# AssemblyAI-Community/MinImagen

Measured on NVIDIA H100. Metric: denoising steps/sec (SR256 U-Net, batch 32 per GPU per step), higher is better.
Workload: dtype f16 tensor-core operands, f32 accumulate / residual stream

## Files before the change

include/minimagen_b200.h:

```cpp
#ifndef MINIMAGEN_B200_H_
#define MINIMAGEN_B200_H_

#include <stdint.h>

#ifdef __cplusplus
extern "C" {
#endif

#define MI_ABI_VERSION 2

int mi_abi_version(void);
const char* mi_last_error(void);
int mi_device_ok(void);
int mi_set_launch_mode(int programmatic_dependent_launch);

int mi_pack_conv_weight_f16(const float* w_oihw, int c_out, int c_in, int kh, int kw, float scale, void* out_f16,
                            void* stream);

int mi_pack_conv_weight_dgrad_f16(const float* w_oihw, int c_out, int c_in, int kh, int kw, void* out_f16, void* stream);

int mi_conv2d_igemm_supported(int H, int W, int c_in, int c_out);
int mi_conv2d_igemm_f16(const void* act_f16, int B, int H, int W, int lda, int c_off, int c_in, const void* act2_f16,
                        int lda2, int c_off2, int c_in1, const void* w_f16, int c_out, int kh, int kw, int mode,
                        const float* bias, const float* residual, float* out_f32, void* out_f16, double* out_stats,
                        long long out_sb, long long out_sh, long long out_sw, long long out_sc, int n_valid,
                        int block_n, int* err_flag, void* workspace, long long workspace_bytes, void* stream);
int mi_conv3x3_res1x1_supported(int H, int W, int c_in, int c_out, int x_cin);
int mi_conv3x3_res1x1_f16(const void* act_f16, int B, int H, int W, int lda, int c_in, const void* act2_f16, int lda2,
                          int c_in1, const void* x_f16, int ldx, int x_cin, const void* x2_f16, int ldx2, int x_cin1,
                          const void* w_f16, int c_out, const float* bias, const float* residual, float* out_f32,
                          void* out_f16, double* out_stats, int* err_flag, void* stream);
long long mi_conv2d_igemm_workspace_bytes(void);

int mi_conv3x3_gn_supported(int H, int W, int c0, int c1, int c_out, int groups);
int mi_conv3x3_gn_silu_f16(const float* src0, int c0, const float* src1, int c1, float scale1, int B, int H, int W,
                           int groups, const double* stats0, const double* stats1, const float* gamma,
                           const float* beta, const float* scale_shift, int scale_shift_ld, float eps,
                           const void* w_f16, int c_out, const float* bias, const float* residual, float* out_f32,
                           void* out_f16, double* out_stats, int* err_flag, void* stream);

int mi_conv2d_direct_f32(const float* in, int B, int Hin, int Win, int c_in, int ldi, const float* w_oihw, int c_out,
                         int kh, int kw, int stride, int pad, const float* bias, const float* residual, float* out,
                         int Hout, int Wout, long long out_sb, long long out_sh, long long out_sw, long long out_sc,
                         void* stream);

int mi_gn_stats(const void* src0, int c0, const void* src1, int c1, float scale1, int in_is_f16, int B, int hw,
                int groups, double* sums, void* stream);
int mi_gn_apply_silu(const void* src0, int c0, const void* src1, int c1, float scale1, int in_is_f16, int B, int hw,
                     int groups, const double* stats0, int stats0_block, const double* stats1, int stats1_block,
                     const float* gamma, const float* beta, const float* scale_shift, int scale_shift_ld, float eps,
                     void* out, int out_is_f16, void* stream);
int mi_cast_act(const void* src0, int c0, const void* src1, int c1, float scale1, int in_is_f16, int B, int H, int W,
                int mode, void* out, int out_is_f16, void* stream);
int mi_ln_rows(const float* in, long long rows, int C, const float* gamma, const float* beta, float eps, int pre_gelu,
               const float* residual, float* out_f32, void* out_f16, void* stream);

int mi_linear_f32(const float* in, int M, int K, const float* W, const float* bias, int N, int in_act, int out_act,
                  const float* addend, float* out_f32, void* out_f16, float out_scale, void* stream);
int mi_sinusoidal_posemb(const long long* t, int B, int dim, float* out, void* stream);
int mi_text_tokens(const float* proj, int B, int L, int D, const uint8_t* mask, const uint8_t* keep,
                   const float* null_embed, int max_len, float* c_out, int m, int row_off, float* pooled,
                   void* stream);
// ... 83 lines not shown
```

minimagen_b200/csrc/capi.cu:

```cuda
#include "../../include/minimagen_b200.h"

#include <cuda_runtime.h>
#include <stdio.h>
#include <stdlib.h>
#include <string.h>
#include <string>

#include "conv_tc.cuh"
#include "kernels.cuh"

namespace {

thread_local char g_err[256] = "ok";

int fail(int code, const char* what) {
    snprintf(g_err, sizeof(g_err), "%s (code %d)", what, code);
    return code;
}
int check(int rc, const char* fn) {
    if (rc == 0) return 0;
    if (rc == -1) return fail(rc, (std::string(fn) + ": unsupported shape / alignment").c_str());
    if (rc == -2) {
        cudaError_t e = cudaGetLastError();
        return fail(rc, (std::string(fn) + ": kernel launch failed: " + cudaGetErrorString(e)).c_str());
    }
    return fail(rc, (std::string(fn) + ": error").c_str());
}
inline cudaStream_t S(void* s) { return reinterpret_cast<cudaStream_t>(s); }

}

namespace mi {
static bool g_pdl = false;
bool pdl_enabled() { return g_pdl; }
}

extern "C" {

int mi_abi_version(void) { return MI_ABI_VERSION; }
int mi_set_launch_mode(int programmatic_dependent_launch) {
    mi::g_pdl = programmatic_dependent_launch != 0;
    return 0;
}
const char* mi_last_error(void) { return g_err; }

int mi_device_ok(void) {
    int dev = 0, major = 0;
    if (cudaGetDevice(&dev) != cudaSuccess) return 0;
    if (cudaDeviceGetAttribute(&major, cudaDevAttrComputeCapabilityMajor, dev) != cudaSuccess) return 0;
    return major == 9;
}

int mi_pack_conv_weight_dgrad_f16(const float* w, int c_out, int c_in, int kh, int kw, void* out, void* stream) {
    return check(mi::pack_conv_weight_dgrad(w, c_out, c_in, kh, kw, (__half*)out, S(stream)), "mi_pack_conv_weight_dgrad_f16");
}
int mi_pack_conv_weight_f16(const float* w, int c_out, int c_in, int kh, int kw, float scale, void* out, void* stream) {
    return check(mi::pack_conv_weight(w, c_out, c_in, kh, kw, scale, (__half*)out, S(stream)), "mi_pack_conv_weight_f16");
}

int mi_conv2d_igemm_supported(int H, int W, int c_in, int c_out) { return mi::conv_tc_supported(H, W, c_in, c_out) ? 1 : 0; }

static int igemm_common(const void* act, int B, int H, int W, int lda, int c_off, int c_in, const void* act2, int lda2,
                        int c_off2, int c_in1, const void* w, int c_out, int kh, int kw, int mode, const float* bias,
                        const float* residual, float* out_f32, void* out_f16, double* out_stats, long long out_sb,
                        long long out_sh, long long out_sw, long long out_sc, int n_valid, int block_n, int* err_flag,
                        void* workspace, long long workspace_bytes, const void* x_act, int ldx, int x_off, int x_cin,
                        const void* x_act2, int ldx2, int x_off2, int x_cin1, void* stream) {
    mi::ConvTcProblem p{};
    p.x_act = x_act; p.x_lda = ldx; p.x_chan_off = x_off; p.Cx = x_cin;
    p.x_act2 = x_act2; p.x_lda2 = ldx2; p.x_chan_off2 = x_off2; p.Cx1 = x_cin1;
    if (x_act && !(mode == 0 && kh == 3 && kw == 3)) return fail(-9, "mi_conv3x3_res1x1_f16: the folded 1x1 operand needs a 3x3 stride-1 conv");
    (void)workspace; (void)workspace_bytes;
    p.act = act; p.B = B; p.H = H; p.W = W; p.lda = lda; p.a_channels = lda; p.a_chan_off = c_off; p.Cin = c_in;
    p.wpacked = w; p.Cout = c_out;
    p.act2 = act2; p.lda2 = lda2; p.a_chan_off2 = c_off2; p.Cin1 = c_in1; p.stats = out_stats;
    if (out_stats && (out_sc > 1 || (c_out % 32) != 0)) return fail(-8, "mi_conv2d_igemm_f16: out_stats needs channel-contiguous output and c_out % 32 == 0");
    if (out_stats && ((long long)H * W) % 32 != 0)
        return fail(-8, "mi_conv2d_igemm_f16: out_stats needs H*W % 32 == 0 (a warp's output rows must belong to one image)");
    p.out_f32 = out_f32; p.out_f16 = (__half*)out_f16; p.bias = bias; p.residual = residual;
    p.out_sb = out_sb; p.out_sh = out_sh; p.out_sw = out_sw; p.out_sc = out_sc; p.n_valid = n_valid;
    p.block_n_hint = block_n; p.err_flag = err_flag;
    if (mode == 0) {
        if (!(kh & 1) || !(kw & 1) || kh * kw > mi::kConvMaxTaps) return fail(-4, "mi_conv2d_igemm_f16: mode 0 needs odd kh,kw with kh*kw <= 16");
// ... 297 lines not shown
```

minimagen_b200/csrc/conv_tc.cu:

```cuda
#include "conv_tc.cuh"

#include <cuda_runtime.h>
#include <mutex>
#include <stdio.h>

#include "kernels.cuh"
#include "launch.cuh"
#include "ptx.cuh"
#include "sat_half.cuh"
#include "wgmma.cuh"

namespace mi {

namespace {

constexpr int kNumThreads = 384;
constexpr uint32_t kABytes = kConvBlockM * kConvBlockK * 2;
constexpr uint32_t kRingBudget = 192 * 1024;
constexpr uint32_t kAuxBytes = 512;
constexpr uint32_t kSmemMax = 227 * 1024;
constexpr int kProducerRegs = 40;
constexpr int kConsumerRegs = 232;
static_assert(128 * kProducerRegs + 256 * kConsumerRegs <= 65536, "register file overcommitted");
constexpr int kTurnBar = 2;
constexpr int kStatBar = 4;
constexpr uint32_t stat_scratch_bytes(int block_n) { return 2 * 4 * (block_n / 16 > 0 ? block_n / 16 : 1) * 2 * 8; }

template <int BLOCK_N>
struct Cfg {
    static constexpr uint32_t kBBytes = BLOCK_N * kConvBlockK * 2;
    static constexpr uint32_t kStageBytes = kABytes + kBBytes;
    static constexpr int kStages = (kRingBudget / kStageBytes) > 8 ? 8 : (kRingBudget / kStageBytes);
    static constexpr uint32_t kSmemBytes = kStages * kStageBytes + 1024  + kAuxBytes;
};

__device__ __forceinline__ float silu(float v) { return __fdividef(v, 1.0f + __expf(-v)); }

template <int BLOCK_N, bool GN>
__global__ void __launch_bounds__(kNumThreads, 1)
conv_wg_kernel(const __grid_constant__ CUtensorMap tmA, const __grid_constant__ CUtensorMap tmA2,
               const __grid_constant__ CUtensorMap tmB, const __grid_constant__ CUtensorMap tmX,
               const __grid_constant__ CUtensorMap tmX2, const __grid_constant__ ConvTcArgs args,
               const __grid_constant__ GnPrologueArgs gn) {
    using C = Cfg<BLOCK_N>;
    constexpr int STAGES = C::kStages;
    static_assert(2 * STAGES * 8 <= 256, "barrier block overlaps the GroupNorm scratch");
    constexpr bool PP = !GN && BLOCK_N <= 128;
    constexpr int HALVES = PP ? 2 : 1;

    extern __shared__ uint8_t smem_raw[];
    uint8_t* smem = reinterpret_cast<uint8_t*>((reinterpret_cast<uintptr_t>(smem_raw) + 1023) & ~uintptr_t(1023));
    uint64_t* bars = reinterpret_cast<uint64_t*>(smem + STAGES * C::kStageBytes);
    uint64_t* full_bar = bars;
    uint64_t* empty_bar = bars + STAGES;

    const int warp = threadIdx.x >> 5;
    const int lane = threadIdx.x & 31;
    const int wg = threadIdx.x >> 7;
    int* err = args.err_flag;

    if (threadIdx.x == 0) {
        ptx::prefetch_tensormap(&tmB);
        if (!GN) {
            ptx::prefetch_tensormap(&tmA);
            ptx::prefetch_tensormap(&tmA2);
        }
        for (int i = 0; i < STAGES; ++i) {
            ptx::mbar_init(&full_bar[i], GN ? 5 : 1);
            ptx::mbar_init(&empty_bar[i], PP ? 1 : 2);
        }
        ptx::fence_barrier_init();
    }
    __syncthreads();
    pdl_wait();

    const int num_tap_kb = args.num_taps * args.chunks_per_tap;
    const int num_kb = num_tap_kb + args.x_chunks;
    const int tiles_m = args.tiles_w * args.tiles_h * args.tiles_b;
    const int total_tiles = tiles_m * args.tiles_n;
    const int BW = 1 << args.bw_log2, BH = 1 << args.bh_log2;
    const int BB = kConvBlockM >> (args.bw_log2 + args.bh_log2);

    if (wg == 0) {
        if constexpr (!GN) {
            ptx::setmaxnreg_dec<kProducerRegs>();
            if (warp == 0) {
                int stage = 0;
                uint32_t phase = 0;
                for (int tile = blockIdx.x; tile < total_tiles; tile += gridDim.x) {
                    const int nt = tile % args.tiles_n;
                    const int mt = tile / args.tiles_n;
                    const int w0 = (mt % args.tiles_w) * BW;
                    const int h0 = ((mt / args.tiles_w) % args.tiles_h) * BH;
                    const int b0 = (mt / (args.tiles_w * args.tiles_h)) * BB;
                    const int n0 = nt * BLOCK_N;
                    for (int kb = 0; kb < num_kb; ++kb) {
                        ptx::mbar_wait(&empty_bar[stage], phase ^ 1, err, 100 + stage);
                        if (ptx::elect_one()) {
                            uint8_t* sa = smem + stage * C::kStageBytes;
                            uint8_t* sb = sa + kABytes;
                            ptx::mbar_arrive_expect_tx(&full_bar[stage], C::kStageBytes);
                            if (kb < num_tap_kb) {
                                const int t = kb / args.chunks_per_tap, j = kb - t * args.chunks_per_tap;
                                const int cw = w0 * args.in_stride + args.dw[t], ch = h0 * args.in_stride + args.dh[t];
                                if (j < args.a_split)
                                    ptx::tma_load_5d(&tmA, &full_bar[stage], sa, args.a_chan_off + j * kConvBlockK, cw, ch,
                                                     args.ph[t], b0);
                                else
                                    ptx::tma_load_5d(&tmA2, &full_bar[stage], sa,
                                                     args.a_chan_off2 + (j - args.a_split) * kConvBlockK, cw, ch, args.ph[t], b0);
                            } else {
                                const int jx = kb - num_tap_kb;
                                if (jx < args.x_split)
                                    ptx::tma_load_5d(&tmX, &full_bar[stage], sa, args.x_chan_off + jx * kConvBlockK, w0, h0, 0, b0);
                                else
                                    ptx::tma_load_5d(&tmX2, &full_bar[stage], sa,
                                                     args.x_chan_off2 + (jx - args.x_split) * kConvBlockK, w0, h0, 0, b0);
                            }
                            ptx::tma_load_2d(&tmB, &full_bar[stage], sb, kb * kConvBlockK, n0);
                        }
                        if (++stage == STAGES) { stage = 0; phase ^= 1; }
                    }
                }
                pdl_trigger();
            }
        } else {
            float* s_mean = reinterpret_cast<float*>(reinterpret_cast<uint8_t*>(bars) + 256);
            float* s_rstd = s_mean + 32;
            float* sA = reinterpret_cast<float*>(reinterpret_cast<uint8_t*>(bars) + kAuxBytes);
            const int tt = threadIdx.x;
            const int lq = tt & 7;
            const int prow = tt >> 3;
            const int C0 = gn.C0, C1 = gn.C1, Ctot = C0 + C1, Cg = Ctot / gn.groups;
            const int H = args.H, W = args.W;
// ... 71 lines not shown
                    float4 x0[8], x1[8];
                    bool ok[8];
#pragma unroll
                    for (int i = 0; i < 8; ++i) {
                        const int m = i * 16 + prow;
                        const int gw = w0 + (m & (BW - 1)) + dw;
                        const int gh = h0 + ((m >> args.bw_log2) & (BH - 1)) + dh;
                        ok[i] = gh >= 0 && gh < H && gw >= 0 && gw < W;
                        if (ok[i]) {
                            const float4* s4 = reinterpret_cast<const float4*>(src + ((long long)gh * W + gw) * Cs);
                            x0[i] = __ldg(s4);
                            x1[i] = __ldg(s4 + 1);
                        }
                    }
#pragma unroll
                    for (int i = 0; i < 8; ++i) {
                        const int m = i * 16 + prow;
                        uint4 o = make_uint4(0u, 0u, 0u, 0u);
                        if (ok[i]) {
                            const __half2 h0_ = sat_half2(silu(fmaf(x0[i].x, a0.x, b0.x)), silu(fmaf(x0[i].y, a0.y, b0.y)));
                            const __half2 h1_ = sat_half2(silu(fmaf(x0[i].z, a0.z, b0.z)), silu(fmaf(x0[i].w, a0.w, b0.w)));
                            const __half2 h2_ = sat_half2(silu(fmaf(x1[i].x, a1.x, b1.x)), silu(fmaf(x1[i].y, a1.y, b1.y)));
                            const __half2 h3_ = sat_half2(silu(fmaf(x1[i].z, a1.z, b1.z)), silu(fmaf(x1[i].w, a1.w, b1.w)));
                            o.x = *reinterpret_cast<const uint32_t*>(&h0_); o.y = *reinterpret_cast<const uint32_t*>(&h1_);
                            o.z = *reinterpret_cast<const uint32_t*>(&h2_); o.w = *reinterpret_cast<const uint32_t*>(&h3_);
                        }
                        *reinterpret_cast<uint4*>(sa + m * 128 + ((lq ^ (m & 7)) << 4)) = o;
                    }
                    ptx::fence_proxy_async_smem();
                    __syncwarp();
                    if (lane == 0) ptx::mbar_arrive(&full_bar[stage]);
                    if (++stage == STAGES) { stage = 0; phase ^= 1; }
                }
            }
            pdl_trigger();
        }
    } else {
        if constexpr (!GN) ptx::setmaxnreg_inc<kConsumerRegs>();
        const int cw = wg - 1;
        const int wq = warp & 3;
        const int cq = 2 * (lane & 3);
        float acc[HALVES][BLOCK_N / 2];
        int stage = 0;
        uint32_t phase = 0;
        auto skip = [&](int n) {
            stage += n % STAGES;
            phase ^= (uint32_t)(n / STAGES) & 1u;
            if (stage >= STAGES) { stage -= STAGES; phase ^= 1; }
        };
        if (PP) skip(cw * num_kb);
        int bw_r[2 * HALVES], bh_r[2 * HALVES], bb_r[2 * HALVES], bb_warp[HALVES];
#pragma unroll
        for (int h = 0; h < HALVES; ++h) {
            const int m_warp = (PP ? h : cw) * 64 + wq * 16;
            bb_warp[h] = m_warp >> (args.bw_log2 + args.bh_log2);
#pragma unroll
            for (int r = 0; r < 2; ++r) {
                const int m = m_warp + (lane >> 2) + 8 * r;
                bw_r[2 * h + r] = m & (BW - 1);
                bh_r[2 * h + r] = (m >> args.bw_log2) & (BH - 1);
                bb_r[2 * h + r] = m >> (args.bw_log2 + args.bh_log2);
            }
        }
        constexpr int NQ = BLOCK_N / 16 > 0 ? BLOCK_N / 16 : 1;
        const bool tile_stats = PP && args.stats != nullptr && BB == 1;
        double* st_red = reinterpret_cast<double*>(reinterpret_cast<uint8_t*>(bars) + kAuxBytes);
        const bool vec = args.out_sc == 1 && ((reinterpret_cast<uintptr_t>(args.out_f32) & 7) == 0) &&
                         ((reinterpret_cast<uintptr_t>(args.residual) & 7) == 0) &&
                         ((reinterpret_cast<uintptr_t>(args.out_f16) & 3) == 0);

        for (int tile = blockIdx.x + (PP ? cw : 0) * gridDim.x; tile < total_tiles; tile += (PP ? 2 : 1) * gridDim.x) {
            const int nt = tile % args.tiles_n;
            const int mt = tile / args.tiles_n;
            const int n0 = nt * BLOCK_N;
            if (PP && tile != (int)blockIdx.x) ptx::bar_sync(kTurnBar + cw, 256);
            int prev = -1;
            for (int kb = 0; kb < num_kb; ++kb) {
                ptx::mbar_wait(&full_bar[stage], phase, err, 300 + stage);
                const uint32_t sa = ptx::smem_u32(smem + stage * C::kStageBytes);
                const uint64_t db = ptx::make_sw128_desc(sa + kABytes);
                ptx::wg_fence();
#pragma unroll
                for (int k = 0; k < kConvBlockK / 16; ++k)
#pragma unroll
                    for (int h = 0; h < HALVES; ++h) {
                        const uint64_t da = ptx::make_sw128_desc(sa + (PP ? h : cw) * (64 * 128));
                        ptx::Wgmma<BLOCK_N, 0>::run(acc[h], da + 2 * k, db + 2 * k, (kb | k) != 0);
                    }
                ptx::wg_commit();
                ptx::wg_wait<1>();
                if (prev >= 0 && (threadIdx.x & 127) == 0) ptx::mbar_arrive(&empty_bar[prev]);
                prev = stage;
                if (++stage == STAGES) { stage = 0; phase ^= 1; }
            }
            if (PP && tile + (int)gridDim.x < total_tiles) ptx::bar_arrive(kTurnBar + (cw ^ 1), 256);
            if (PP) skip(num_kb);
            ptx::wg_wait<0>();
#pragma unroll
            for (int h = 0; h < HALVES; ++h) ptx::wg_fence_regs(acc[h]);
            if (prev >= 0 && (threadIdx.x & 127) == 0) ptx::mbar_arrive(&empty_bar[prev]);

            const int tw0 = (mt % args.tiles_w) * BW;
            const int th0 = ((mt / args.tiles_w) % args.tiles_h) * BH;
            const int tb0 = (mt / (args.tiles_w * args.tiles_h)) * BB;
            const bool fast = vec && n0 + BLOCK_N <= args.n_valid;
#pragma unroll
            for (int hf = 0; hf < HALVES; ++hf) {
                bool valid[2];
                long long pix[2];
#pragma unroll
                for (int r = 0; r < 2; ++r) {
                    const int w = tw0 + bw_r[2 * hf + r], h = th0 + bh_r[2 * hf + r], b = tb0 + bb_r[2 * hf + r];
                    valid[r] = (b < args.B) && (h < args.H) && (w < args.W);
                    pix[r] = (long long)b * args.out_sb + (long long)h * args.out_sh + (long long)w * args.out_sw;
                }
                const float* a = acc[hf];
                float st_s[BLOCK_N / 16 > 0 ? BLOCK_N / 16 : 1], st_q[BLOCK_N / 16 > 0 ? BLOCK_N / 16 : 1];
#pragma unroll
                for (int q = 0; q < BLOCK_N / 16; ++q) { st_s[q] = 0.f; st_q[q] = 0.f; }
#pragma unroll
                for (int j = 0; j < BLOCK_N / 8; ++j) {
                    const int n = n0 + 8 * j + cq;
                    if (fast) {
                        float2 bv = make_float2(0.f, 0.f);
                        if (args.bias) bv = __ldg(reinterpret_cast<const float2*>(args.bias + n));
#pragma unroll
                        for (int r = 0; r < 2; ++r) {
                            if (!valid[r]) continue;
                            const long long o = pix[r] + n;
                            float2 f = make_float2(a[4 * j + 2 * r] + bv.x, a[4 * j + 2 * r + 1] + bv.y);
                            if (args.residual) {
                                const float2 rv = *reinterpret_cast<const float2*>(args.residual + o);
                                f.x += rv.x; f.y += rv.y;
                            }
                            st_s[j >> 1] += f.x + f.y;
                            st_q[j >> 1] += f.x * f.x + f.y * f.y;
                            if (args.out_f32) *reinterpret_cast<float2*>(args.out_f32 + o) = f;
                            if (args.out_f16) *reinterpret_cast<__half2*>(args.out_f16 + o) = sat_half2(f.x, f.y);
                        }
// ... 38 lines not shown
            }
            if (tile_stats) {
                ptx::bar_sync(kStatBar + cw, 128);
                if (wq == 0 && lane < NQ) {
                    const double* r = st_red + (cw * 4 * NQ + lane) * 2;
                    double s = r[0], sq = r[1];
#pragma unroll
                    for (int w = 1; w < 4; ++w) { s += r[w * NQ * 2]; sq += r[w * NQ * 2 + 1]; }
                    double* dst = args.stats + ((long long)tb0 * args.stats_blocks + (n0 >> 4) + lane) * 2;
                    atomicAdd(dst, s);
                    atomicAdd(dst + 1, sq);
                }
                ptx::bar_sync(kStatBar + cw, 128);
            }
        }
    }
}


typedef CUresult (*PFN_encodeTiled)(CUtensorMap*, CUtensorMapDataType, cuuint32_t, void*, const cuuint64_t*,
                                    const cuuint64_t*, const cuuint32_t*, const cuuint32_t*, CUtensorMapInterleave,
                                    CUtensorMapSwizzle, CUtensorMapL2promotion, CUtensorMapFloatOOBfill);

PFN_encodeTiled get_encode() {
    static PFN_encodeTiled fn = nullptr;
    static std::once_flag once;
    std::call_once(once, [] {
        void* p = nullptr;
        cudaDriverEntryPointQueryResult q;
        if (cudaGetDriverEntryPoint("cuTensorMapEncodeTiled", &p, cudaEnableDefault, &q) == cudaSuccess &&
            q == cudaDriverEntryPointSuccess)
            fn = reinterpret_cast<PFN_encodeTiled>(p);
    });
    return fn;
}

int ilog2_exact(int v) {
    int l = 0;
    while ((1 << l) < v) ++l;
    return ((1 << l) == v) ? l : -1;
}

int num_sms_of_current_device() {
    int dev = 0;
    cudaGetDevice(&dev);
    static int cache[64] = {0};
    if (dev < 64 && cache[dev] != 0) return cache[dev];
    int n = 0;
    cudaDeviceGetAttribute(&n, cudaDevAttrMultiProcessorCount, dev);
    if (dev < 64) cache[dev] = n;
    return n;
}

void tile_geometry(int H, int W, int B, ConvTcArgs& a) {
    int BW = W >= 128 ? 128 : W;
    int BH = 128 / BW;
    if (BH > H) BH = H;
    const int BB = 128 / (BW * BH);
    a.bw_log2 = ilog2_exact(BW);
    a.bh_log2 = ilog2_exact(BH);
    a.tiles_w = (W + BW - 1) / BW;
    a.tiles_h = H / BH;
    a.tiles_b = (B + BB - 1) / BB;
    a.B = B; a.H = H; a.W = W;
}

int pick_block_n(int Cout, int tiles_m, int hint, int num_sms) {
    const int cands[5] = {256, 128, 64, 32, 16};
    if (hint < 0) hint = -hint;
    if (hint > 0 && Cout % hint == 0)
        for (int i = 0; i < 5; ++i)
            if (cands[i] == hint) return hint;
    int block_n = 16;
    for (int i = 0; i < 5; ++i) {
        if (Cout % cands[i] != 0) continue;
        block_n = cands[i];
        if (tiles_m * (Cout / cands[i]) >= num_sms || cands[i] <= 64) break;
    }
    return block_n;
}

CUresult encode_act(PFN_encodeTiled enc, CUtensorMap* m, const void* ptr, cuuint64_t channels, cuuint64_t ld, int W, int H,
                    int phases, int B, int in_stride, const ConvTcArgs& a) {
    const cuuint64_t IS = in_stride;
    const int BW = 1 << a.bw_log2, BH = 1 << a.bh_log2, BB = kConvBlockM >> (a.bw_log2 + a.bh_log2);
    cuuint64_t gdim[5] = {channels, (cuuint64_t)W * IS, (cuuint64_t)H * IS, (cuuint64_t)phases, (cuuint64_t)B};
    cuuint64_t gstr[4] = {ld * 2, (cuuint64_t)W * IS * ld * 2, (cuuint64_t)H * IS * W * IS * ld * 2,
                          (cuuint64_t)phases * H * IS * W * IS * ld * 2};
    cuuint32_t box[5] = {kConvBlockK, (cuuint32_t)(BW * IS), (cuuint32_t)(BH * IS), 1, (cuuint32_t)BB};
    cuuint32_t estr[5] = {1, (cuuint32_t)IS, (cuuint32_t)IS, 1, 1};
    return enc(m, CU_TENSOR_MAP_DATA_TYPE_FLOAT16, 5, const_cast<void*>(ptr), gdim, gstr, box, estr,
               CU_TENSOR_MAP_INTERLEAVE_NONE, CU_TENSOR_MAP_SWIZZLE_128B, CU_TENSOR_MAP_L2_PROMOTION_L2_256B,
               CU_TENSOR_MAP_FLOAT_OOB_FILL_NONE);
}

CUresult encode_weights(PFN_encodeTiled enc, CUtensorMap* m, const void* ptr, cuuint64_t K, int Cout, int block_n) {
    cuuint64_t gdim[2] = {K, (cuuint64_t)Cout};
    cuuint64_t gstr[1] = {K * 2};
    cuuint32_t box[2] = {kConvBlockK, (cuuint32_t)block_n};
    cuuint32_t estr[2] = {1, 1};
    return enc(m, CU_TENSOR_MAP_DATA_TYPE_FLOAT16, 2, const_cast<void*>(ptr), gdim, gstr, box, estr,
               CU_TENSOR_MAP_INTERLEAVE_NONE, CU_TENSOR_MAP_SWIZZLE_128B, CU_TENSOR_MAP_L2_PROMOTION_L2_256B,
               CU_TENSOR_MAP_FLOAT_OOB_FILL_NONE);
}

template <int BLOCK_N, bool GN>
int launch(const CUtensorMap& tmA, const CUtensorMap& tmA2, const CUtensorMap& tmB, const CUtensorMap& tmX,
           const CUtensorMap& tmX2, const ConvTcArgs& args, const GnPrologueArgs& gn, uint32_t extra_smem,
           cudaStream_t stream) {
    using C = Cfg<BLOCK_N>;
    static bool attr_set = false;
    if (!attr_set) {
        if (cudaFuncSetAttribute(conv_wg_kernel<BLOCK_N, GN>, cudaFuncAttributeMaxDynamicSharedMemorySize, kSmemMax) !=
            cudaSuccess)
            return -10;
        attr_set = true;
    }
    const int total_tiles = args.tiles_w * args.tiles_h * args.tiles_b * args.tiles_n;
    const int num_sms = num_sms_of_current_device();
    const int grid = total_tiles < num_sms ? total_tiles : num_sms;
    const uint32_t smem = C::kSmemBytes + (!GN && BLOCK_N <= 128 ? stat_scratch_bytes(BLOCK_N) : 0u) + extra_smem;
    launch_k(conv_wg_kernel<BLOCK_N, GN>, grid, kNumThreads, smem, stream, tmA, tmA2, tmB, tmX, tmX2, args, gn);
    return cudaGetLastError() == cudaSuccess ? 0 : -11;
}

}

PFN_tmaEncodeTiled get_tma_encode() { return get_encode(); }

const char* conv_tc_strerror(int code) {
    switch (code) {
        case 0: return "ok";
        case -1: return "conv_tc: C_in (per tap) must be a positive multiple of 64";
        case -2: return "conv_tc: C_out must be a multiple of 16";
        case -3: return "conv_tc: W must be a power of two >= 8 or a multiple of 128; H*W tiling unsupported";
        case -4: return "conv_tc: too many taps (max 16)";
        case -5: return "conv_tc: cuTensorMapEncodeTiled unavailable";
        case -6: return "conv_tc: tensor map encode failed (activations)";
        case -7: return "conv_tc: tensor map encode failed (weights)";
        case -8: return "conv_tc: pointer/stride alignment (16 B) violated";
        case -9: return "conv_tc: the folded 1x1 operand needs a stride-1 conv over one phase";
        case -10: return "conv_tc: cudaFuncSetAttribute(max dynamic smem) failed";
        case -11: return "conv_tc: kernel launch failed";
        default: return "conv_tc: unknown error";
    }
}

bool conv_tc_supported(int H, int W, int Cin, int Cout) {
    if (Cin <= 0 || Cin % kConvBlockK != 0 || Cout <= 0 || Cout % 16 != 0) return false;
    if (W >= 128) return true;
    if (ilog2_exact(W) < 3) return false;
    const int bh = 128 / W;
    if (H >= bh) return H % bh == 0;
    return ilog2_exact(H) >= 0;
}

int conv_tc_launch(const ConvTcProblem& p, cudaStream_t stream) {
    if (p.Cin <= 0 || p.Cin % kConvBlockK != 0) return -1;
    if (p.Cout % 16 != 0) return -2;
    if (p.num_taps < 1 || p.num_taps > kConvMaxTaps) return -4;
    if (!conv_tc_supported(p.H, p.W, p.Cin, p.Cout)) return -3;
    if ((reinterpret_cast<uintptr_t>(p.act) & 15) || (reinterpret_cast<uintptr_t>(p.wpacked) & 15) ||
        (p.lda % 8) != 0)
        return -8;
    PFN_encodeTiled enc = get_encode();
    if (!enc) return -5;

    ConvTcArgs a{};
    a.num_taps = p.num_taps;
    a.chunks_per_tap = p.Cin / kConvBlockK;
    tile_geometry(p.H, p.W, p.B, a);
    a.a_chan_off = p.a_chan_off;
    a.in_stride = p.in_stride == 2 ? 2 : 1;
    a.out_sb = p.out_sb; a.out_sh = p.out_sh; a.out_sw = p.out_sw;
    a.out_sc = p.out_sc > 0 ? p.out_sc : 1;
    a.n_valid = p.n_valid > 0 ? p.n_valid : p.Cout;
    a.out_f32 = p.out_f32; a.out_f16 = p.out_f16; a.bias = p.bias; a.residual = p.residual;
    a.err_flag = p.err_flag;
    a.stats = p.stats; a.stats_blocks = p.Cout / 16;
    for (int t = 0; t < p.num_taps; ++t) { a.dh[t] = p.dh[t]; a.dw[t] = p.dw[t]; a.ph[t] = p.ph[t]; }

    const int tiles_m = a.tiles_w * a.tiles_h * a.tiles_b;
    const int block_n = pick_block_n(p.Cout, tiles_m, p.block_n_hint, num_sms_of_current_device());
    a.tiles_n = p.Cout / block_n;

    CUtensorMap tmA, tmA2, tmB, tmX, tmX2;
    a.a_split = (p.act2 ? p.Cin1 : p.Cin) / kConvBlockK;
    a.a_chan_off2 = p.a_chan_off2;
    if (encode_act(enc, &tmA, p.act, p.a_channels, p.lda, p.W, p.H, p.phases, p.B, a.in_stride, a) != CUDA_SUCCESS) return -6;
    tmA2 = tmA;
    if (p.act2) {
        if (p.Cin1 <= 0 || p.Cin1 % kConvBlockK || p.Cin1 >= p.Cin || (p.lda2 % 8) || (reinterpret_cast<uintptr_t>(p.act2) & 15) ||
            a.in_stride != 1)
            return -8;
        if (encode_act(enc, &tmA2, p.act2, p.lda2, p.lda2, p.W, p.H, p.phases, p.B, 1, a) != CUDA_SUCCESS) return -6;
    }
    tmX = tmA; tmX2 = tmA;
    if (p.x_act) {
        if (p.phases != 1 || a.in_stride != 1) return -9;
        if (p.Cx <= 0 || p.Cx % kConvBlockK || (p.x_lda % 8) || (reinterpret_cast<uintptr_t>(p.x_act) & 15)) return -8;
        if (p.x_act2 && (p.Cx1 <= 0 || p.Cx1 % kConvBlockK || p.Cx1 >= p.Cx || (p.x_lda2 % 8) ||
                         (reinterpret_cast<uintptr_t>(p.x_act2) & 15)))
            return -8;
        a.x_chunks = p.Cx / kConvBlockK;
        a.x_split = (p.x_act2 ? p.Cx1 : p.Cx) / kConvBlockK;
        a.x_chan_off = p.x_chan_off; a.x_chan_off2 = p.x_chan_off2;
        if (encode_act(enc, &tmX, p.x_act, p.x_lda, p.x_lda, p.W, p.H, 1, p.B, 1, a) != CUDA_SUCCESS) return -6;
        tmX2 = tmX;
        if (p.x_act2 && encode_act(enc, &tmX2, p.x_act2, p.x_lda2, p.x_lda2, p.W, p.H, 1, p.B, 1, a) != CUDA_SUCCESS) return -6;
    }
    const cuuint64_t K = (cuuint64_t)p.num_taps * p.Cin + (p.x_act ? (cuuint64_t)p.Cx : 0);
    if (encode_weights(enc, &tmB, p.wpacked, K, p.Cout, block_n) != CUDA_SUCCESS) return -7;

    const GnPrologueArgs gn{};
    switch (block_n) {
        case 256: return launch<256, false>(tmA, tmA2, tmB, tmX, tmX2, a, gn, 0, stream);
        case 128: return launch<128, false>(tmA, tmA2, tmB, tmX, tmX2, a, gn, 0, stream);
        case 64: return launch<64, false>(tmA, tmA2, tmB, tmX, tmX2, a, gn, 0, stream);
        case 32: return launch<32, false>(tmA, tmA2, tmB, tmX, tmX2, a, gn, 0, stream);
        default: return launch<16, false>(tmA, tmA2, tmB, tmX, tmX2, a, gn, 0, stream);
    }
}


bool conv_gn_supported(int H, int W, int C0, int C1, int Cout, int groups) {
    const int C = C0 + C1;
    if (H <= 0 || W <= 0 || H % 32 || W % 8 || C0 <= 0 || C0 % 64 || C1 < 0 || C1 % 64 || Cout <= 0 || Cout % 128) return false;
    if (!conv_tc_supported(H, W, C, Cout) || H * W < kConvBlockM) return false;
    if (groups < 1 || groups > 32 || C % groups) return false;
    if (Cfg<128>::kSmemBytes + 8u * (uint32_t)C > kSmemMax) return false;
    return (C / groups) % 16 == 0;
}

int conv_gn_launch(const ConvGnProblem& p, cudaStream_t stream) {
    if (!conv_gn_supported(p.H, p.W, p.C0, p.C1, p.Cout, p.groups)) return -3;
    if (p.C1 && (!p.src1 || !p.stats1)) return -8;
    if (!p.src0 || !p.stats0 || !p.gamma || !p.beta) return -8;
    if ((reinterpret_cast<uintptr_t>(p.src0) & 15) || (reinterpret_cast<uintptr_t>(p.src1) & 15) ||
        (reinterpret_cast<uintptr_t>(p.wpacked) & 15))
        return -8;
    PFN_encodeTiled enc = get_encode();
    if (!enc) return -5;
    const int C = p.C0 + p.C1;

    ConvTcArgs a{};
    a.num_taps = 9;
    for (int t = 0; t < 9; ++t) { a.dh[t] = (int8_t)(t / 3 - 1); a.dw[t] = (int8_t)(t % 3 - 1); a.ph[t] = 0; }
    a.chunks_per_tap = C / kConvBlockK;
    a.a_split = p.C0 / kConvBlockK;
    a.in_stride = 1;
    tile_geometry(p.H, p.W, p.B, a);
    a.out_sb = (long long)p.H * p.W * p.Cout; a.out_sh = (long long)p.W * p.Cout; a.out_sw = p.Cout; a.out_sc = 1;
    a.n_valid = p.Cout;
    a.out_f32 = p.out_f32; a.out_f16 = p.out_f16; a.bias = p.bias; a.residual = p.residual; a.err_flag = p.err_flag;
    a.stats = p.out_stats; a.stats_blocks = p.Cout / 16;
    a.tiles_n = p.Cout / 128;

    GnPrologueArgs g{};
    g.src0 = p.src0; g.src1 = p.src1;
    g.C0 = p.C0; g.C1 = p.C1; g.groups = p.groups; g.scale1 = p.scale1; g.eps = p.eps;
    g.stats0 = p.stats0; g.stats1 = p.stats1; g.gamma = p.gamma; g.beta = p.beta;
    g.scale_shift = p.scale_shift; g.ss_ld = p.ss_ld;

    CUtensorMap tmB;
    if (encode_weights(enc, &tmB, p.wpacked, (cuuint64_t)9 * C, p.Cout, 128) != CUDA_SUCCESS) return -7;
    return launch<128, true>(tmB, tmB, tmB, tmB, tmB, a, g, 8u * (uint32_t)C, stream);
}

}
```

minimagen_b200/csrc/conv_tc.cuh:

```cuda
#pragma once
#include <cuda_fp16.h>
#include <cuda_runtime.h>
#include <stdint.h>

namespace mi {

constexpr int kConvBlockM = 128;
constexpr int kConvBlockK = 64;
constexpr int kConvMaxTaps = 16;

struct ConvTcArgs {
    int num_taps, chunks_per_tap;
    int bw_log2, bh_log2;
    int tiles_w, tiles_h, tiles_b, tiles_n;
    int B, H, W;
    int a_chan_off;
    int in_stride;
    int a_split, a_chan_off2;
    int x_chunks, x_split;
    int x_chan_off, x_chan_off2;
    long long out_sb, out_sh, out_sw;
    long long out_sc;
    int n_valid;
    float* out_f32;
    __half* out_f16;
    const float* bias;
    const float* residual;
    int* err_flag;
    double* stats;
    int stats_blocks;
    int8_t dh[kConvMaxTaps], dw[kConvMaxTaps], ph[kConvMaxTaps];
};

struct ConvTcProblem {
    const void* act;
    int B, H, W;
    int phases;
    int in_stride;
    int lda;
    int a_channels;
    int a_chan_off;
    int Cin;
    const void* act2;
    int lda2, a_chan_off2, Cin1;
    const void* wpacked;
    int Cout;
    const void* x_act; int x_lda, x_chan_off, Cx;
    const void* x_act2; int x_lda2, x_chan_off2, Cx1;
    int num_taps;
    int8_t dh[kConvMaxTaps], dw[kConvMaxTaps], ph[kConvMaxTaps];
    float* out_f32; __half* out_f16; const float* bias; const float* residual;
    long long out_sb, out_sh, out_sw;
    long long out_sc;
    int n_valid;
    int block_n_hint;
    double* stats;
    int* err_flag;
};

struct GnPrologueArgs {
    const float* src0;
    const float* src1;
// ... 32 lines not shown
```

minimagen_b200/ops.py:

```python
import torch

from . import _native as N

F16, F32, F64, I64, U8 = torch.float16, torch.float32, torch.float64, torch.int64, torch.uint8


def _chk(t, dtype, name):
    if t is None:
        return
    if t.dtype != dtype:
        raise TypeError(f"{name}: expected {dtype}, got {t.dtype}")
    if not t.is_contiguous():
        raise ValueError(f"{name}: tensor must be contiguous")


def _chk_out(t, dtype, name):
    if t is not None and t.dtype != dtype:
        raise TypeError(f"{name}: expected {dtype}, got {t.dtype}")


class NativeOps:
    name = "native-sm90a"
    attention_tc = True

    def set_launch_mode(self, pdl):
        N.load().mi_set_launch_mode(int(bool(pdl)))

    def igemm_supported(self, H, W, c_in, c_out):
        return bool(N.load().mi_conv2d_igemm_supported(int(H), int(W), int(c_in), int(c_out)))

    def pack_conv_weight(self, w, scale=1.0):
        if w.dim() == 2:
            w = w[:, :, None, None]
        w = w.detach().to(F32).contiguous()
        O, I, KH, KW = w.shape
        out = torch.empty((O, KH * KW * I), dtype=F16, device=w.device)
        N.call("mi_pack_conv_weight_f16", N.ptr(w), O, I, KH, KW, float(scale), N.ptr(out), N.stream())
        return out

    def pack_conv_weight_dgrad(self, w):
        if w.dim() == 2:
            w = w[:, :, None, None]
        w = w.detach().to(F32).contiguous()
        O, I, KH, KW = w.shape
        out = torch.empty((I, KH * KW * O), dtype=F16, device=w.device)
        N.call("mi_pack_conv_weight_dgrad_f16", N.ptr(w), O, I, KH, KW, N.ptr(out), N.stream())
        return out

    def conv_igemm(self, act, B, H, W, lda, c_off, c_in, wp, c_out, kh, kw, mode, bias, residual, out_f32, out_f16,
                   out_strides, block_n=0, out_sc=1, n_valid=0, act2=None, lda2=0, c_off2=0, c_in1=0, out_stats=None):
        _chk(act, F16, "act"); _chk(act2, F16, "act2"); _chk(wp, F16, "wp"); _chk(bias, F32, "bias")
        _chk_out(residual, F32, "residual"); _chk_out(out_f32, F32, "out_f32"); _chk_out(out_f16, F16, "out_f16")
        _chk(out_stats, F64, "out_stats")
        sb, sh, sw = out_strides
        N.call("mi_conv2d_igemm_f16", N.ptr(act), B, H, W, lda, c_off, c_in, N.ptr(act2), lda2, c_off2, c_in1,
               N.ptr(wp), c_out, kh, kw, mode, N.ptr(bias), N.ptr(residual), N.ptr(out_f32), N.ptr(out_f16),
               N.ptr(out_stats), sb, sh, sw, out_sc, n_valid, block_n, None, None, 0, N.stream())
# ... 301 lines not shown
```

Baseline: 15.67.

## Add opt-in 256-pixel M tile to conv kernel and avoid wide N tiles for short K

Templates the implicit-GEMM conv kernel on BLOCK_M and adds a 256-row tile variant with BLOCK_N=128. In that variant both consumer warpgroups each own two 64-row halves, so every weight tile loaded into shared memory feeds twice as many rows. The variant is selected only when a new flag bit is set in the block_n hint, and the Python side only defines the constant without passing it. Separately, the block_n heuristic now skips 256-wide N tiles when the K loop is short (36 or fewer k-blocks). That change applies by default and trades wider tiles for more tiles and less pipeline fill overhead on short-K convs. The 256-row tile also shrinks the ring-stage count because each stage is larger.

Result: no change. 15.74 (median of 6 runs) (+0.4%).

```diff
diff --git a/include/minimagen_b200.h b/include/minimagen_b200.h
--- a/include/minimagen_b200.h
+++ b/include/minimagen_b200.h
@@ -8,6 +8,7 @@
 #endif
 
 #define MI_ABI_VERSION 2
+#define MI_CONV_TILE_M256 0x10000
 
 int mi_abi_version(void);
 const char* mi_last_error(void);
diff --git a/minimagen_b200/csrc/capi.cu b/minimagen_b200/csrc/capi.cu
--- a/minimagen_b200/csrc/capi.cu
+++ b/minimagen_b200/csrc/capi.cu
@@ -29,6 +29,8 @@
 inline cudaStream_t S(void* s) { return reinterpret_cast<cudaStream_t>(s); }
 
 }
+
+static_assert(mi::kConvTileM256 == MI_CONV_TILE_M256, "block_n tile flag of the C ABI");
 
 namespace mi {
 static bool g_pdl = false;
diff --git a/minimagen_b200/csrc/conv_tc.cu b/minimagen_b200/csrc/conv_tc.cu
--- a/minimagen_b200/csrc/conv_tc.cu
+++ b/minimagen_b200/csrc/conv_tc.cu
@@ -15,7 +15,6 @@
 namespace {
 
 constexpr int kNumThreads = 384;
-constexpr uint32_t kABytes = kConvBlockM * kConvBlockK * 2;
 constexpr uint32_t kRingBudget = 192 * 1024;
 constexpr uint32_t kAuxBytes = 512;
 constexpr uint32_t kSmemMax = 227 * 1024;
@@ -26,8 +25,9 @@
 constexpr int kStatBar = 4;
 constexpr uint32_t stat_scratch_bytes(int block_n) { return 2 * 4 * (block_n / 16 > 0 ? block_n / 16 : 1) * 2 * 8; }
 
-template <int BLOCK_N>
+template <int BLOCK_N, int BLOCK_M>
 struct Cfg {
+    static constexpr uint32_t kABytes = BLOCK_M * kConvBlockK * 2;
     static constexpr uint32_t kBBytes = BLOCK_N * kConvBlockK * 2;
     static constexpr uint32_t kStageBytes = kABytes + kBBytes;
     static constexpr int kStages = (kRingBudget / kStageBytes) > 8 ? 8 : (kRingBudget / kStageBytes);
@@ -36,17 +36,20 @@
 
 __device__ __forceinline__ float silu(float v) { return __fdividef(v, 1.0f + __expf(-v)); }
 
-template <int BLOCK_N, bool GN>
+template <int BLOCK_N, int BLOCK_M, bool GN>
 __global__ void __launch_bounds__(kNumThreads, 1)
 conv_wg_kernel(const __grid_constant__ CUtensorMap tmA, const __grid_constant__ CUtensorMap tmA2,
                const __grid_constant__ CUtensorMap tmB, const __grid_constant__ CUtensorMap tmX,
                const __grid_constant__ CUtensorMap tmX2, const __grid_constant__ ConvTcArgs args,
                const __grid_constant__ GnPrologueArgs gn) {
-    using C = Cfg<BLOCK_N>;
+    using C = Cfg<BLOCK_N, BLOCK_M>;
+    constexpr uint32_t kABytes = C::kABytes;
     constexpr int STAGES = C::kStages;
     static_assert(2 * STAGES * 8 <= 256, "barrier block overlaps the GroupNorm scratch");
-    constexpr bool PP = !GN && BLOCK_N <= 128;
-    constexpr int HALVES = PP ? 2 : 1;
+    static_assert(BLOCK_M == 128 || (BLOCK_M == 256 && BLOCK_N == 128 && !GN), "256-pixel tiles are 128 wide, TMA-fed");
+    constexpr bool PP = !GN && BLOCK_N <= 128 && BLOCK_M == 128;
+    constexpr int HALVES = PP || BLOCK_M == 256 ? 2 : 1;
+    constexpr int CONS_ROWS = PP ? 0 : BLOCK_M / 2;
 
     extern __shared__ uint8_t smem_raw[];
     uint8_t* smem = reinterpret_cast<uint8_t*>((reinterpret_cast<uintptr_t>(smem_raw) + 1023) & ~uintptr_t(1023));
@@ -79,7 +82,7 @@
     const int tiles_m = args.tiles_w * args.tiles_h * args.tiles_b;
     const int total_tiles = tiles_m * args.tiles_n;
     const int BW = 1 << args.bw_log2, BH = 1 << args.bh_log2;
-    const int BB = kConvBlockM >> (args.bw_log2 + args.bh_log2);
+    const int BB = BLOCK_M >> (args.bw_log2 + args.bh_log2);
 
     if (wg == 0) {
         if constexpr (!GN) {
@@ -257,7 +260,7 @@
         int bw_r[2 * HALVES], bh_r[2 * HALVES], bb_r[2 * HALVES], bb_warp[HALVES];
 #pragma unroll
         for (int h = 0; h < HALVES; ++h) {
-            const int m_warp = (PP ? h : cw) * 64 + wq * 16;
+            const int m_warp = cw * CONS_ROWS + h * 64 + wq * 16;
             bb_warp[h] = m_warp >> (args.bw_log2 + args.bh_log2);
 #pragma unroll
             for (int r = 0; r < 2; ++r) {
@@ -268,7 +271,7 @@
             }
         }
         constexpr int NQ = BLOCK_N / 16 > 0 ? BLOCK_N / 16 : 1;
-        const bool tile_stats = PP && args.stats != nullptr && BB == 1;
+        const bool tile_stats = HALVES == 2 && args.stats != nullptr && BB == 1;
         double* st_red = reinterpret_cast<double*>(reinterpret_cast<uint8_t*>(bars) + kAuxBytes);
         const bool vec = args.out_sc == 1 && ((reinterpret_cast<uintptr_t>(args.out_f32) & 7) == 0) &&
                          ((reinterpret_cast<uintptr_t>(args.residual) & 7) == 0) &&
@@ -289,7 +292,7 @@
                 for (int k = 0; k < kConvBlockK / 16; ++k)
 #pragma unroll
                     for (int h = 0; h < HALVES; ++h) {
-                        const uint64_t da = ptx::make_sw128_desc(sa + (PP ? h : cw) * (64 * 128));
+                        const uint64_t da = ptx::make_sw128_desc(sa + (cw * CONS_ROWS + h * 64) * 128);
                         ptx::Wgmma<BLOCK_N, 0>::run(acc[h], da + 2 * k, db + 2 * k, (kb | k) != 0);
                     }
                 ptx::wg_commit();
@@ -434,11 +437,18 @@
     return n;
 }
 
-void tile_geometry(int H, int W, int B, ConvTcArgs& a) {
+bool tile_fits(int H, int W, int block_m) {
+    if (W < 128 && ilog2_exact(W) < 3) return false;
+    const int bh = block_m / (W >= 128 ? 128 : W);
+    if (H >= bh) return H % bh == 0;
+    return ilog2_exact(H) >= 0;
+}
+
+void tile_geometry(int H, int W, int B, int block_m, ConvTcArgs& a) {
     int BW = W >= 128 ? 128 : W;
-    int BH = 128 / BW;
+    int BH = block_m / BW;
     if (BH > H) BH = H;
-    const int BB = 128 / (BW * BH);
+    const int BB = block_m / (BW * BH);
     a.bw_log2 = ilog2_exact(BW);
     a.bh_log2 = ilog2_exact(BH);
     a.tiles_w = (W + BW - 1) / BW;
@@ -447,25 +457,32 @@
     a.B = B; a.H = H; a.W = W;
 }
 
-int pick_block_n(int Cout, int tiles_m, int hint, int num_sms) {
+constexpr int kShortKb = 36;
+int pick_block_n(int Cout, int tiles_m, int num_kb, int hint, int num_sms) {
     const int cands[5] = {256, 128, 64, 32, 16};
     if (hint < 0) hint = -hint;
+    hint &= ~kConvTileM256;
     if (hint > 0 && Cout % hint == 0)
         for (int i = 0; i < 5; ++i)
             if (cands[i] == hint) return hint;
     int block_n = 16;
     for (int i = 0; i < 5; ++i) {
-        if (Cout % cands[i] != 0) continue;
+        if (Cout % cands[i] != 0 || (cands[i] == 256 && num_kb <= kShortKb)) continue;
         block_n = cands[i];
         if (tiles_m * (Cout / cands[i]) >= num_sms || cands[i] <= 64) break;
     }
     return block_n;
 }
 
+int pick_block_m(int block_n, int hint) {
+    if (hint < 0) hint = -hint;
+    return block_n == 128 && (hint & kConvTileM256) ? 256 : 128;
+}
+
 CUresult encode_act(PFN_encodeTiled enc, CUtensorMap* m, const void* ptr, cuuint64_t channels, cuuint64_t ld, int W, int H,
-                    int phases, int B, int in_stride, const ConvTcArgs& a) {
+                    int phases, int B, int in_stride, int block_m, const ConvTcArgs& a) {
     const cuuint64_t IS = in_stride;
-    const int BW = 1 << a.bw_log2, BH = 1 << a.bh_log2, BB = kConvBlockM >> (a.bw_log2 + a.bh_log2);
+    const int BW = 1 << a.bw_log2, BH = 1 << a.bh_log2, BB = block_m >> (a.bw_log2 + a.bh_log2);
     cuuint64_t gdim[5] = {channels, (cuuint64_t)W * IS, (cuuint64_t)H * IS, (cuuint64_t)phases, (cuuint64_t)B};
     cuuint64_t gstr[4] = {ld * 2, (cuuint64_t)W * IS * ld * 2, (cuuint64_t)H * IS * W * IS * ld * 2,
                           (cuuint64_t)phases * H * IS * W * IS * ld * 2};
@@ -486,14 +503,14 @@
                CU_TENSOR_MAP_FLOAT_OOB_FILL_NONE);
 }
 
-template <int BLOCK_N, bool GN>
+template <int BLOCK_N, int BLOCK_M, bool GN>
 int launch(const CUtensorMap& tmA, const CUtensorMap& tmA2, const CUtensorMap& tmB, const CUtensorMap& tmX,
            const CUtensorMap& tmX2, const ConvTcArgs& args, const GnPrologueArgs& gn, uint32_t extra_smem,
            cudaStream_t stream) {
-    using C = Cfg<BLOCK_N>;
+    using C = Cfg<BLOCK_N, BLOCK_M>;
     static bool attr_set = false;
     if (!attr_set) {
-        if (cudaFuncSetAttribute(conv_wg_kernel<BLOCK_N, GN>, cudaFuncAttributeMaxDynamicSharedMemorySize, kSmemMax) !=
+        if (cudaFuncSetAttribute(conv_wg_kernel<BLOCK_N, BLOCK_M, GN>, cudaFuncAttributeMaxDynamicSharedMemorySize, kSmemMax) !=
             cudaSuccess)
             return -10;
         attr_set = true;
@@ -502,7 +519,7 @@
     const int num_sms = num_sms_of_current_device();
     const int grid = total_tiles < num_sms ? total_tiles : num_sms;
     const uint32_t smem = C::kSmemBytes + (!GN && BLOCK_N <= 128 ? stat_scratch_bytes(BLOCK_N) : 0u) + extra_smem;
-    launch_k(conv_wg_kernel<BLOCK_N, GN>, grid, kNumThreads, smem, stream, tmA, tmA2, tmB, tmX, tmX2, args, gn);
+    launch_k(conv_wg_kernel<BLOCK_N, BLOCK_M, GN>, grid, kNumThreads, smem, stream, tmA, tmA2, tmB, tmX, tmX2, args, gn);
     return cudaGetLastError() == cudaSuccess ? 0 : -11;
 }
 
@@ -530,11 +547,7 @@
 
 bool conv_tc_supported(int H, int W, int Cin, int Cout) {
     if (Cin <= 0 || Cin % kConvBlockK != 0 || Cout <= 0 || Cout % 16 != 0) return false;
-    if (W >= 128) return true;
-    if (ilog2_exact(W) < 3) return false;
-    const int bh = 128 / W;
-    if (H >= bh) return H % bh == 0;
-    return ilog2_exact(H) >= 0;
+    return tile_fits(H, W, kConvBlockM);
 }
 
 int conv_tc_launch(const ConvTcProblem& p, cudaStream_t stream) {
@@ -551,7 +564,7 @@
     ConvTcArgs a{};
     a.num_taps = p.num_taps;
     a.chunks_per_tap = p.Cin / kConvBlockK;
-    tile_geometry(p.H, p.W, p.B, a);
+    tile_geometry(p.H, p.W, p.B, kConvBlockM, a);
     a.a_chan_off = p.a_chan_off;
     a.in_stride = p.in_stride == 2 ? 2 : 1;
     a.out_sb = p.out_sb; a.out_sh = p.out_sh; a.out_sw = p.out_sw;
@@ -563,19 +576,26 @@
     for (int t = 0; t < p.num_taps; ++t) { a.dh[t] = p.dh[t]; a.dw[t] = p.dw[t]; a.ph[t] = p.ph[t]; }
 
     const int tiles_m = a.tiles_w * a.tiles_h * a.tiles_b;
-    const int block_n = pick_block_n(p.Cout, tiles_m, p.block_n_hint, num_sms_of_current_device());
+    const int num_kb = p.num_taps * (p.Cin / kConvBlockK) + (p.x_act ? p.Cx / kConvBlockK : 0);
+    const int block_n = pick_block_n(p.Cout, tiles_m, num_kb, p.block_n_hint, num_sms_of_current_device());
+    const int block_m = pick_block_m(block_n, p.block_n_hint);
+    if (block_m != kConvBlockM) {
+        if (!tile_fits(p.H, p.W, block_m)) return -3;
+        tile_geometry(p.H, p.W, p.B, block_m, a);
+    }
     a.tiles_n = p.Cout / block_n;
 
     CUtensorMap tmA, tmA2, tmB, tmX, tmX2;
     a.a_split = (p.act2 ? p.Cin1 : p.Cin) / kConvBlockK;
     a.a_chan_off2 = p.a_chan_off2;
-    if (encode_act(enc, &tmA, p.act, p.a_channels, p.lda, p.W, p.H, p.phases, p.B, a.in_stride, a) != CUDA_SUCCESS) return -6;
+    if (encode_act(enc, &tmA, p.act, p.a_channels, p.lda, p.W, p.H, p.phases, p.B, a.in_stride, block_m, a) != CUDA_SUCCESS)
+        return -6;
     tmA2 = tmA;
     if (p.act2) {
         if (p.Cin1 <= 0 || p.Cin1 % kConvBlockK || p.Cin1 >= p.Cin || (p.lda2 % 8) || (reinterpret_cast<uintptr_t>(p.act2) & 15) ||
             a.in_stride != 1)
             return -8;
-        if (encode_act(enc, &tmA2, p.act2, p.lda2, p.lda2, p.W, p.H, p.phases, p.B, 1, a) != CUDA_SUCCESS) return -6;
+        if (encode_act(enc, &tmA2, p.act2, p.lda2, p.lda2, p.W, p.H, p.phases, p.B, 1, block_m, a) != CUDA_SUCCESS) return -6;
     }
     tmX = tmA; tmX2 = tmA;
     if (p.x_act) {
@@ -587,20 +607,23 @@
         a.x_chunks = p.Cx / kConvBlockK;
         a.x_split = (p.x_act2 ? p.Cx1 : p.Cx) / kConvBlockK;
         a.x_chan_off = p.x_chan_off; a.x_chan_off2 = p.x_chan_off2;
-        if (encode_act(enc, &tmX, p.x_act, p.x_lda, p.x_lda, p.W, p.H, 1, p.B, 1, a) != CUDA_SUCCESS) return -6;
+        if (encode_act(enc, &tmX, p.x_act, p.x_lda, p.x_lda, p.W, p.H, 1, p.B, 1, block_m, a) != CUDA_SUCCESS) return -6;
         tmX2 = tmX;
-        if (p.x_act2 && encode_act(enc, &tmX2, p.x_act2, p.x_lda2, p.x_lda2, p.W, p.H, 1, p.B, 1, a) != CUDA_SUCCESS) return -6;
+        if (p.x_act2 &&
+            encode_act(enc, &tmX2, p.x_act2, p.x_lda2, p.x_lda2, p.W, p.H, 1, p.B, 1, block_m, a) != CUDA_SUCCESS)
+            return -6;
     }
     const cuuint64_t K = (cuuint64_t)p.num_taps * p.Cin + (p.x_act ? (cuuint64_t)p.Cx : 0);
     if (encode_weights(enc, &tmB, p.wpacked, K, p.Cout, block_n) != CUDA_SUCCESS) return -7;
 
     const GnPrologueArgs gn{};
+    if (block_m == 256) return launch<128, 256, false>(tmA, tmA2, tmB, tmX, tmX2, a, gn, 0, stream);
     switch (block_n) {
-        case 256: return launch<256, false>(tmA, tmA2, tmB, tmX, tmX2, a, gn, 0, stream);
-        case 128: return launch<128, false>(tmA, tmA2, tmB, tmX, tmX2, a, gn, 0, stream);
-        case 64: return launch<64, false>(tmA, tmA2, tmB, tmX, tmX2, a, gn, 0, stream);
-        case 32: return launch<32, false>(tmA, tmA2, tmB, tmX, tmX2, a, gn, 0, stream);
-        default: return launch<16, false>(tmA, tmA2, tmB, tmX, tmX2, a, gn, 0, stream);
+        case 256: return launch<256, 128, false>(tmA, tmA2, tmB, tmX, tmX2, a, gn, 0, stream);
+        case 128: return launch<128, 128, false>(tmA, tmA2, tmB, tmX, tmX2, a, gn, 0, stream);
+        case 64: return launch<64, 128, false>(tmA, tmA2, tmB, tmX, tmX2, a, gn, 0, stream);
+        case 32: return launch<32, 128, false>(tmA, tmA2, tmB, tmX, tmX2, a, gn, 0, stream);
+        default: return launch<16, 128, false>(tmA, tmA2, tmB, tmX, tmX2, a, gn, 0, stream);
     }
 }
 
@@ -610,7 +633,7 @@
     if (H <= 0 || W <= 0 || H % 32 || W % 8 || C0 <= 0 || C0 % 64 || C1 < 0 || C1 % 64 || Cout <= 0 || Cout % 128) return false;
     if (!conv_tc_supported(H, W, C, Cout) || H * W < kConvBlockM) return false;
     if (groups < 1 || groups > 32 || C % groups) return false;
-    if (Cfg<128>::kSmemBytes + 8u * (uint32_t)C > kSmemMax) return false;
+    if (Cfg<128, 128>::kSmemBytes + 8u * (uint32_t)C > kSmemMax) return false;
     return (C / groups) % 16 == 0;
 }
 
@@ -631,7 +654,7 @@
     a.chunks_per_tap = C / kConvBlockK;
     a.a_split = p.C0 / kConvBlockK;
     a.in_stride = 1;
-    tile_geometry(p.H, p.W, p.B, a);
+    tile_geometry(p.H, p.W, p.B, kConvBlockM, a);
     a.out_sb = (long long)p.H * p.W * p.Cout; a.out_sh = (long long)p.W * p.Cout; a.out_sw = p.Cout; a.out_sc = 1;
     a.n_valid = p.Cout;
     a.out_f32 = p.out_f32; a.out_f16 = p.out_f16; a.bias = p.bias; a.residual = p.residual; a.err_flag = p.err_flag;
@@ -646,7 +669,7 @@
 
     CUtensorMap tmB;
     if (encode_weights(enc, &tmB, p.wpacked, (cuuint64_t)9 * C, p.Cout, 128) != CUDA_SUCCESS) return -7;
-    return launch<128, true>(tmB, tmB, tmB, tmB, tmB, a, g, 8u * (uint32_t)C, stream);
-}
-
-}
+    return launch<128, 128, true>(tmB, tmB, tmB, tmB, tmB, a, g, 8u * (uint32_t)C, stream);
+}
+
+}
diff --git a/minimagen_b200/csrc/conv_tc.cuh b/minimagen_b200/csrc/conv_tc.cuh
--- a/minimagen_b200/csrc/conv_tc.cuh
+++ b/minimagen_b200/csrc/conv_tc.cuh
@@ -8,6 +8,7 @@
 constexpr int kConvBlockM = 128;
 constexpr int kConvBlockK = 64;
 constexpr int kConvMaxTaps = 16;
+constexpr int kConvTileM256 = 1 << 16;
 
 struct ConvTcArgs {
     int num_taps, chunks_per_tap;
diff --git a/minimagen_b200/ops.py b/minimagen_b200/ops.py
--- a/minimagen_b200/ops.py
+++ b/minimagen_b200/ops.py
@@ -3,6 +3,7 @@
 from . import _native as N
 
 F16, F32, F64, I64, U8 = torch.float16, torch.float32, torch.float64, torch.int64, torch.uint8
+CONV_TILE_M256 = 0x10000
 
 
 def _chk(t, dtype, name):
```
